# icameling/lidar_camera_calibration

Hardware: AMD Instinct MI355X
Metric: chessboard-corner frames/sec + max corner error (mm), VLP-16 cloud (higher is better)
Workload: dtype f32

## Files before the change

### include/ilcc_hip.h

```cpp
#ifndef ILCC_HIP_H_
#define ILCC_HIP_H_

#include <stdint.h>

#ifdef __cplusplus
extern "C" {
#endif

#define ILCC_MAX_CORNERS 256
#define ILCC_ABI_VERSION 5

enum {
  ILCC_OK = 0,
  ILCC_NO_ROI_POINTS = 1,
  ILCC_NO_CLUSTER = 2,
  ILCC_NO_PLANE = 3,
  ILCC_DEGENERATE_HIST = 4,
  ILCC_TOO_FEW_POINTS = 5,
  ILCC_BAD_ARGUMENT = 6,
  ILCC_CAPACITY = 7,
  ILCC_HIP_ERROR = 8,
  ILCC_IO_ERROR = 9,
  ILCC_BOARD_NOT_FOUND = 10,
  ILCC_AMBIGUOUS = 11
// ... 151 lines not shown
int64_t ilcc_fetch_walk(ilcc_handle* h, uint32_t frame, float* out_yz, uint8_t* out_label, uint64_t cap_points,
                        uint32_t counts[2]);

int32_t ilcc_grid_cost(ilcc_handle* h, const float* yz, const uint8_t* label, uint32_t m,
                       int32_t use_oob, float* cost_out, int32_t* best_index, float* best_cost);

int32_t ilcc_grid_solve(ilcc_handle* h, const float* yz, const uint8_t* label, uint32_t m, int32_t* grid_index, float* grid_cost,
                        int32_t lat[3], int32_t* phase, int64_t* cost_q, int64_t* alt_cost_q, int32_t* rounds, int32_t* hops,
                        int32_t* flags, int32_t* ties);

int32_t ilcc_pattern_refine(ilcc_handle* h, const float* yz, const uint8_t* label, uint32_t m, int32_t lat[3],
                            int32_t* phase, int64_t* cost_q, int64_t* alt_cost_q, int32_t* rounds, int32_t* hops);

int32_t ilcc_get_theta_t(ilcc_handle* h, const float* yz, const uint8_t* label, uint32_t m,
                         int32_t topleft_white, int32_t use_oob, double theta_t[3], double* cost,
                         int32_t* iterations);

#define ILCC_SOLVE_REC_DOUBLES 6
#define ILCC_SOLVE_REC_INTS 4
int32_t ilcc_debug_reference_solve(ilcc_handle* h, const float* yz, const uint8_t* label, const uint64_t* offsets,
                                   const int32_t* status_in, uint32_t n_frames, double* rec_f64, int32_t* rec_i32,
                                   ilcc_result* results, uint32_t* lds_points);

#define ILCC_TIMELINE_COLS 15
int32_t ilcc_debug_timeline_enable(ilcc_handle* h, int32_t on);
int32_t ilcc_debug_timeline_fetch(ilcc_handle* h, double* rows, uint32_t cap_rows);

int32_t ilcc_debug_separate_launches(ilcc_handle* h, int32_t on);

#define ILCC_CLUSTER_HOME_RULE 0
#define ILCC_CLUSTER_HOME_LDS 1
#define ILCC_CLUSTER_HOME_L2 2
#define ILCC_CLUSTER_LAUNCH_WORDS 6
int32_t ilcc_debug_cluster_home(ilcc_handle* h, int32_t home);
int32_t ilcc_debug_cluster_launch(const ilcc_handle* h, uint32_t out[ILCC_CLUSTER_LAUNCH_WORDS]);

int32_t ilcc_debug_group_prepass(ilcc_handle* h, uint32_t* states_out, uint32_t* mask_out, uint32_t dims_out[2], uint32_t* bound_out);
int64_t ilcc_debug_solve_walk(ilcc_handle* h, float* out_yz, uint8_t* out_label, uint64_t cap_points, uint32_t counts[2]);

void ilcc_get_timing(const ilcc_handle* h, ilcc_timing* t);
void ilcc_reset_timing(ilcc_handle* h);

int32_t ilcc_save_corners2txt(const float* corners_xyz, uint32_t n_corners, const char* filename);
int32_t ilcc_read_lidar_corners(const char* filename, uint32_t num, double* out_xyz);

#ifdef __cplusplus
// ... 4 lines not shown
```

### lidar_camera_calibration_amd/_native.py

```python
from __future__ import annotations

import ctypes as C
import os

import numpy as np

_HERE = os.path.dirname(os.path.abspath(__file__))
LIB_PATH = os.environ.get("ILCC_HIP_LIB") or os.path.join(_HERE, "libilcc_hip.so")
MAX_CORNERS = 256

OK, NO_ROI_POINTS, NO_CLUSTER, NO_PLANE, DEGENERATE_HIST, TOO_FEW_POINTS, BAD_ARGUMENT, CAPACITY, \
    HIP_ERROR, IO_ERROR, BOARD_NOT_FOUND, AMBIGUOUS = range(12)
FLAG_TIE_OVERFLOW, FLAG_REFINE_CAPPED, FLAG_LOW_COVERAGE, FLAG_BORDER_RISK = 1, 2, 4, 8
FLAGS_FP32_ONLY = FLAG_TIE_OVERFLOW | FLAG_BORDER_RISK
RECORD_HEADER = 20
TIMELINE_COLS = 15
COST_Q_ONE = float(1 << 40)
SOLVER_REFERENCE_LOCAL, SOLVER_GRID = 0, 1
CLOUD_ROI, CLOUD_CLUSTER, CLOUD_CHESSBOARD, CLOUD_PCA, CLOUD_OPTIM = range(5)

EXPORTS = [
    "ilcc_abi_version", "ilcc_strerror", "ilcc_last_error", "ilcc_default_params",
    "ilcc_set_chessboard_param", "ilcc_create", "ilcc_destroy", "ilcc_set_params", "ilcc_reserve", "ilcc_extract",
    "ilcc_extract_batch", "ilcc_extract_batch_device", "ilcc_submit_batch_device", "ilcc_submit_batch", "ilcc_wait", "ilcc_wait_records_device", "ilcc_fetch_cloud", "ilcc_fetch_labelled", "ilcc_fetch_walk", "ilcc_chessboard_by_point_batch", "ilcc_submit_chessboard_by_point", "ilcc_wait_chessboard_by_point", "ilcc_fetch_classes",
    "ilcc_grid_cost", "ilcc_grid_solve", "ilcc_pattern_refine", "ilcc_get_theta_t", "ilcc_get_timing", "ilcc_reset_timing",
    "ilcc_save_corners2txt", "ilcc_read_lidar_corners",
    "ilcc_set_result_mode", "ilcc_wait_compact", "ilcc_record_floats", "ilcc_fetch_results",
    "ilcc_debug_timeline_enable", "ilcc_debug_timeline_fetch", "ilcc_debug_separate_launches",
    "ilcc_debug_cluster_home", "ilcc_debug_cluster_launch", "ilcc_debug_reference_solve",
    "ilcc_debug_group_prepass", "ilcc_debug_solve_walk",
]
ABI_VERSION = 5
RESULTS_FULL, RESULTS_COMPACT = 0, 1
CLUSTER_HOME_RULE, CLUSTER_HOME_LDS, CLUSTER_HOME_L2 = 0, 1, 2
CLUSTER_LAUNCH_WORDS = 6
SOLVE_REC_DOUBLES, SOLVE_REC_INTS = 6, 4


class Params(C.Structure):
    _fields_ = [
        ("roi_half", C.c_double * 3),
        ("cluster_tol", C.c_double),
        ("cluster_min", C.c_int32),
        ("cluster_max", C.c_int32),
        ("ransac_thresh", C.c_double),
        ("ransac_hyp", C.c_int32),
        ("ransac_seed", C.c_uint32),
        ("hist_bins", C.c_int32),
        ("gray_rate", C.c_double),
        ("huber_delta", C.c_double),
        ("grid_length", C.c_double),
        ("board_w", C.c_int32),
        ("board_h", C.c_int32),
# ... 152 lines not shown
        L.ilcc_wait_compact.restype = C.c_int32
        L.ilcc_record_floats.argtypes = [vp, C.c_int32]
        L.ilcc_record_floats.restype = C.c_uint32
        L.ilcc_debug_timeline_enable.argtypes = [vp, C.c_int32]
        L.ilcc_debug_timeline_enable.restype = C.c_int32
        L.ilcc_debug_timeline_fetch.argtypes = [vp, C.POINTER(C.c_double), C.c_uint32]
        L.ilcc_debug_timeline_fetch.restype = C.c_int32
        if hasattr(L, "ilcc_debug_separate_launches"):
            L.ilcc_debug_separate_launches.argtypes = [vp, C.c_int32]
            L.ilcc_debug_separate_launches.restype = C.c_int32
        if hasattr(L, "ilcc_debug_cluster_home"):
            L.ilcc_debug_cluster_home.argtypes = [vp, C.c_int32]
            L.ilcc_debug_cluster_home.restype = C.c_int32
            L.ilcc_debug_cluster_launch.argtypes = [vp, C.POINTER(C.c_uint32)]
            L.ilcc_debug_cluster_launch.restype = C.c_int32
        L.ilcc_debug_reference_solve.argtypes = [vp, fp, C.POINTER(C.c_uint8), C.POINTER(C.c_uint64), C.POINTER(C.c_int32), C.c_uint32,
                                                 C.POINTER(C.c_double), C.POINTER(C.c_int32), rp, C.POINTER(C.c_uint32)]
        L.ilcc_debug_reference_solve.restype = C.c_int32
        if hasattr(L, "ilcc_debug_group_prepass"):
            L.ilcc_debug_group_prepass.argtypes = [vp, C.POINTER(C.c_uint32), C.POINTER(C.c_uint32), C.POINTER(C.c_uint32), C.POINTER(C.c_uint32)]
            L.ilcc_debug_group_prepass.restype = C.c_int32
            L.ilcc_debug_solve_walk.argtypes = [vp, fp, C.POINTER(C.c_uint8), C.c_uint64, C.POINTER(C.c_uint32)]
            L.ilcc_debug_solve_walk.restype = C.c_int64
        L.ilcc_fetch_results.argtypes = [vp, C.c_uint32, C.c_uint32, rp]
        L.ilcc_fetch_results.restype = C.c_int32
        _lib = L
    return _lib


def default_params() -> Params:
    p = Params()
    lib().ilcc_default_params(C.byref(p))
    return p


def strerror(status: int) -> str:
    return lib().ilcc_strerror(int(status)).decode()


def fptr(a: np.ndarray):
    return a.ctypes.data_as(C.POINTER(C.c_float))
```

### lidar_camera_calibration_amd/csrc/ilcc_api.cpp

```cpp
#include <hip/hip_runtime.h>

#include <array>
#include <cmath>
#include <cstdio>
#include <cstdlib>
#include <cstring>
#include <mutex>
#include <new>
#include <string>
#include <vector>

#include "ilcc_internal.h"
#include "k15_seed.h"
#include "k6_common.h"
#include "k7_common.h"

using namespace ilcc;

namespace ilcc {
bool params_ok(const ilcc_params& p, std::string& why);
}

#ifndef ILCC_SLOTS
#define ILCC_SLOTS 4
// ... 551 lines not shown

GridPass anchor_pass(const ilcc_handle* h, const Ctx& c, const GridSeed& seed, GridPartial* out) {
  GridPass g = whole_grid_pass(c, h->grid, out);
  g.seed = seed;
  g.radius_th = kAnchorRadius;
  g.blocks = 2 * kAnchorRadius + 1;
  return g;
}

GridPass full_pass(const ilcc_handle* h, const Ctx& c, const GridSeed& seed) {
  GridPass g = whole_grid_pass(c, h->grid, c.partial);
  g.seed = seed;
  g.collect_ties = 1u;
  return g;
}

LocatePlan locate_plan(const ilcc_handle* h, const Slot& sl, const Ctx& c) {
  LocatePlan lp{};
  lp.seed = h->seed_grid;
  lp.map = h->seed_map;
  lp.refine_radius = std::max(1, h->seed_map.stride_th / ILCC_REFINE_RADIUS_DIV);
  lp.sample_min = (uint32_t)ILCC_SEED_POINTS;
  lp.sample_cap = std::max((uint32_t)ILCC_SEED_POINTS, ((c.grid_lds_points >> 3) + 63u) & ~63u);
  lp.out = sl.d_partial4;
  return lp;
}

int32_t enqueue_locate_launches(ilcc_handle* h, Slot& sl, const Ctx& c, hipStream_t s, int32_t refine_radius, GridSeed& located) {
  launch_grid_cost(c, seed_pass(h, sl, c), s, 1, nullptr, true);
  HIP_TRY(h, hipEventRecord(sl.ev[kEvSeeded], s));
  const GridPass refine = refine_pass(h, sl, c, refine_radius);
  launch_grid_cost(c, refine, s, 1, nullptr, true);
  HIP_TRY(h, hipEventRecord(sl.ev[kEvRefined], s));
  located = full_table_records(refine.out, refine.blocks);
  GridPartial* const ping[2] = {sl.d_partial4, sl.d_partial2};
  for (int round = 0; round < kAnchorRounds; ++round) {
    const GridPass anchor = anchor_pass(h, c, located, ping[round & 1]);
    launch_anchor(c, anchor, s);
    located = full_table_records(anchor.out, anchor.blocks);
  }
  return ILCC_OK;
}

int32_t enqueue_grid_search(ilcc_handle* h, Slot& sl, const Ctx& c, hipStream_t s, uint32_t n_frames, bool chain, bool walk_laid_out = false) {
  const bool prune = h->p.grid_prune != 0;
  if (!walk_laid_out) launch_walk_order(c, s);
  HIP_TRY(h, hipEventRecord(sl.ev[kEvWalkOrdered], s));
  GridSeed located{};
  if (h->seed_grid.n_th > 0 && h->p.n_th >= 8 && h->p.n_ty >= 8 && h->p.n_tz >= 8) {
    const LocatePlan lp = locate_plan(h, sl, c);
    const bool fused = n_frames >= (uint32_t)kLocateMinFrames && lp.seed.n_th <= 16 &&
                       locate_lds_bytes(lp.sample_cap, h->grid.n_ty, h->grid.n_tz, lp.seed.n_ty, lp.seed.n_tz) <= (size_t)kLocateLdsMax;
    if (fused) {
      launch_locate(c, s, lp);
      HIP_TRY(h, hipEventRecord(sl.ev[kEvSeeded], s));
      HIP_TRY(h, hipEventRecord(sl.ev[kEvRefined], s));
      located = full_table_records(lp.out, 1);
    } else {
      ILCC_TRY(enqueue_locate_launches(h, sl, c, s, lp.refine_radius, located));
    }
  } else {
    HIP_TRY(h, hipEventRecord(sl.ev[kEvSeeded], s));
    HIP_TRY(h, hipEventRecord(sl.ev[kEvRefined], s));
  }
  HIP_TRY(h, hipEventRecord(sl.ev[kEvAnchored], s));
  GridPass full = full_pass(h, c, located);
  const GroupPrepassPlan gp = group_prepass_plan(h->p);
  full.box_points = gp.box ? (uint32_t)ILCC_BOX_POINTS : 0u;
  if (full.box_points != 0u && gp.on && (size_t)n_frames * gp.groups <= sl.grp_alive_cap &&
      (size_t)n_frames * gp.groups * gp.words <= sl.grp_mask_cap) {
    full.grp_alive = sl.d_grp_alive;
    full.grp_mask = sl.d_grp_mask;
    full.grp_count = gp.groups;
    full.grp_words = gp.words;
    launch_group_prepass(c, full, s);
// ... 835 lines not shown
    HIP_TRY(h, hipMemcpyAsync(sl.d_lab, label, total, hipMemcpyHostToDevice, s));
  }
  HIP_TRY(h, hipMemsetAsync(sl.d_solverec, 0xFF, sizeof(SolveRec) * 2 * n_frames, s));
  sl.n_frames = 0;
  const Ctx c = make_ctx(h, sl, nullptr, nullptr, n_frames, 1);
  launch_reference_solve(c, s);
  launch_corners(c, s, solve_slots(c.p));
  HIP_TRY(h, hipGetLastError());
  std::vector<SolveRec> rec(2 * (size_t)n_frames);
  HIP_TRY(h, hipMemcpyAsync(rec.data(), sl.d_solverec, sizeof(SolveRec) * rec.size(), hipMemcpyDeviceToHost, s));
  HIP_TRY(h, hipMemcpyAsync(results, sl.d_res, sizeof(ilcc_result) * n_frames, hipMemcpyDeviceToHost, s));
  ILCC_TRY(sync_own(h, s));
  for (size_t k = 0; k < rec.size(); ++k) {
    const SolveRec& r = rec[k];
    const double d[ILCC_SOLVE_REC_DOUBLES] = {r.x[0], r.x[1], r.x[2], r.cost_a, r.cost_b, r.sel};
    const int32_t i[ILCC_SOLVE_REC_INTS] = {r.iters_a, r.iters_b, r.phase, r.valid};
    std::memcpy(rec_f64 + ILCC_SOLVE_REC_DOUBLES * k, d, sizeof(d));
    std::memcpy(rec_i32 + ILCC_SOLVE_REC_INTS * k, i, sizeof(i));
  }
  if (lds_points) *lds_points = c.grid_lds_points;
  return ILCC_OK;
}

int32_t ilcc_pattern_refine(ilcc_handle* h, const float* yz, const uint8_t* label, uint32_t m, int32_t lat[3],
                            int32_t* phase, int64_t* cost_q, int64_t* alt_cost_q, int32_t* rounds, int32_t* hops) {
  if (!h || !lat || !phase) return ILCC_BAD_ARGUMENT;
  if (lat[0] < h->th_lat_lo || lat[0] > h->th_lat_hi || (*phase != 0 && *phase != 1)) {
    h->err = "ilcc_pattern_refine: theta lattice coordinate outside [th_min - refine_th_margin, th_max + refine_th_margin] steps";
    return ILCC_BAD_ARGUMENT;
  }
  const hipStream_t s = h->stream[take_stream(h)];
  ILCC_TRY(stage_labelled(h, s, yz, label, m));
  Slot& sl = h->slots[0];
  RefineOut io{};
  io.lat[0] = lat[0];
  io.lat[1] = lat[1];
  io.lat[2] = lat[2];
  io.phase = *phase;
  HIP_TRY(h, hipMemcpyAsync(h->d_refine_io, &io, sizeof(io), hipMemcpyHostToDevice, s));
  const Ctx c = diagnostic_ctx(h, sl, 0);
  launch_pattern_refine_test(c, s, h->d_refine_io);
  HIP_TRY(h, hipGetLastError());
  HIP_TRY(h, hipMemcpyAsync(&io, h->d_refine_io, sizeof(io), hipMemcpyDeviceToHost, s));
  ILCC_TRY(sync_own(h, s));
  lat[0] = io.lat[0];
  lat[1] = io.lat[1];
// ... 98 lines not shown
```

### lidar_camera_calibration_amd/csrc/ilcc_internal.h

```cpp
#pragma once

#include <hip/hip_runtime.h>
#include <stdint.h>

#include "ilcc_hip.h"

#define ILCC_WAVE 64

namespace ilcc {

constexpr int kCuLdsBytes = 160 * 1024;
constexpr int kClusterLdsMax = kCuLdsBytes - 4 * 1024;
constexpr int kLocateLdsMax = 3 * (kCuLdsBytes / 8);
constexpr int kSolveLdsMax = kCuLdsBytes - 16 * 1024;

constexpr int kCropThreads = 256;
constexpr int kCropChunk = 4096;
#ifndef ILCC_K2_THREADS
#define ILCC_K2_THREADS 256
#endif
constexpr int kFrameThreads = ILCC_K2_THREADS;
#ifndef ILCC_K3_THREADS
#define ILCC_K3_THREADS 256
#endif
// ... 221 lines not shown
__device__ __forceinline__ uint32_t block_rank(bool flag, uint32_t* scratch, uint32_t& total) {
  const unsigned long long m = __ballot(flag);
  const int lane = lane_id();
  const uint32_t in_wave = __popcll(m & ((1ull << lane) - 1ull));
  const int nw = (blockDim.x + ILCC_WAVE - 1) / ILCC_WAVE;
  __syncthreads();
  if (lane == 0) scratch[wave_id()] = __popcll(m);
  __syncthreads();
  uint32_t base = 0, tot = 0;
  for (int w = 0; w < nw; ++w) {
    const uint32_t c = scratch[w];
    if (w < wave_id()) base += c;
    tot += c;
  }
  total = tot;
  return base + in_wave;
}

struct LocatePlan {
  GridTables seed;
  SeedMap map;
  int32_t refine_radius;
  uint32_t sample_min, sample_cap;
  GridPartial* out;
};

size_t locate_lds_bytes(uint32_t sample_cap, int n_ty, int n_tz, int n_ty2, int n_tz2);
void launch_locate(const Ctx& c, hipStream_t s, const LocatePlan& lp);
void launch_anchor(const Ctx& c, const GridPass& pass, hipStream_t s);
constexpr int kRefineThetaStride = 2;
constexpr int kLocateMinFrames = 512;

void launch_roi_crop(const Ctx& c, hipStream_t s, hipEvent_t after_count = nullptr, bool one_pass = false);
constexpr int kCropFrameMinFrames = 512;
constexpr int32_t kClusterHomeRule = 0, kClusterHomeLds = 1, kClusterHomeL2 = 2;
struct ClusterLimits {
  uint32_t cus, lds_per_cu, threads_per_cu, static_lds;
};
struct ClusterLaunch {
  int32_t home;
  uint32_t lds_bytes, threads;
};
hipError_t cluster_limits(int device, ClusterLimits* out);
ClusterLaunch launch_cluster(const Ctx& c, hipStream_t s, const ClusterLimits& lim, int32_t home);
void launch_cluster_listed(const Ctx& c, hipStream_t s);
constexpr size_t kListedFrameBytes = 64;
hipError_t set_kernel_attributes_k2();
size_t cluster_lds_bytes(uint32_t pts_cap, uint32_t cells_cap, uint32_t bits);
uint32_t cluster_bits_default();
uint32_t cluster_bits_online();
// ... 25 lines not shown
```

### lidar_camera_calibration_amd/csrc/k6_locate.hip

```cpp
#include "k6_common.h"

namespace ilcc {

__device__ __forceinline__ void anchor_walk(const ilcc_params& p, const GridTables& t, const FrameWalk& fw, int k, int a_org, int b_org, const float* ty, const float* tz,
                                            uint32_t part, uint32_t n_parts, float (*s_part)[2], uint32_t& pts_done, uint32_t& pts_in) {
  const int my_s = lane_id() & (kSlices - 1), my_c = lane_id() >> 2;
  const float Wh = 0.5f * (float)p.board_w, Hh = 0.5f * (float)p.board_h, delta2 = (float)p.huber_delta;
  const float cth = t.cth[k], sth = t.sth[k];
  const float ay = ty[min(a_org + (my_c >> 2), t.n_ty - 1)], az = tz[min(b_org + (my_c & 3), t.n_tz - 1)];
  float A0 = 0.f, A1 = 0.f;
  uint32_t pos = 0, pin = 0;
  for (uint32_t at0 = part * kSlices; at0 < fw.M; at0 += n_parts * kSlices) {
    const uint32_t at = at0 + (uint32_t)my_s;
    if (at < fw.M) {
      const uint32_t src = fw.source(at, fw.Mi_all, fw.n_rim_all);
      const float2 v = rotate(fw.yz[src], cth, sth);
      const PointTerms pt{v.x, v.y, fw.lab[src] ? 0.5f : 0.f};
      if (at < fw.Mi_all)
        accumulate_interior(pt, ay, az, delta2, A0, A1);
      else
        accumulate<true>(pt, ay, az, Wh, Hh, delta2, A0, A1);
    }
    pos += kSlices;
    pin += at0 < fw.Mi_all ? (uint32_t)kSlices : 0u;
  }
  pts_done += pos;
  pts_in += pin;
  const float t0s = quad_sum(A0), t1s = quad_sum(A1);
  if (my_s == 0) {
    s_part[my_c][0] = t0s;
    s_part[my_c][1] = t1s;
  }
}

template <int THETAS, int PARTS>
__device__ __forceinline__ void anchor_publish(const GridTables& t, uint32_t* bound, const float (*s_part)[16][2], int k0, int a_org, int b_org,
                                               GridPartial* out) {
  const int lane = lane_id();
  const int n_ty = t.n_ty, n_tz = t.n_tz;
  Best best{__builtin_inff(), 0xFFFFFFFFu, 0xFFFFFFFFu};
  uint32_t ab = 0;
  if (lane < 16 * THETAS) {
    const int th = lane >> 4, cand = lane & 15;
    const int k = min(max(k0 + th, 0), t.n_th - 1), ja = a_org + (cand >> 2), jb = b_org + (cand & 3);
    if (ja < n_ty && jb < n_tz) {
      float h0 = 0.f, h1 = 0.f;
#pragma unroll
      for (int q = 0; q < PARTS; ++q) {
        h0 += s_part[th * PARTS + q][cand][0];
        h1 += s_part[th * PARTS + q][cand][1];
      }
      score(2.f * h0, 2.f * h1, k, ja, jb, n_ty, n_tz, t.c_th, t.c_ty, t.c_tz, best, ab);
    }
  }
  best = wave_argmin<true>(best, ab);
  if (lane == 0) {
    *out = GridPartial{best.cost, best.d2, best.flat, ab};
    if (best.flat != 0xFFFFFFFFu) atomicMin(bound, __float_as_uint(best.cost));
  }
}

constexpr int kLocateThreads = 384;
constexpr int kSeedPeek = 16;
constexpr int kAnchorThetas = 3;
constexpr int kAnchorParts = (kLocateThreads / 64) / kAnchorThetas;
constexpr int kLocateWaves = kLocateThreads / ILCC_WAVE;
constexpr int kLocateThetasMax = 16;
constexpr int kLocateWindowTiles = 2;

struct LocateLds {
  size_t hw, rot, ay, az, ay2, az2, bytes;
};
__host__ __device__ constexpr LocateLds locate_lds(uint32_t sample_cap, int n_ty, int n_tz, int n_ty2, int n_tz2) {
  LocateLds l{};
  l.hw = sizeof(float2) * (size_t)sample_cap;
  l.rot = l.hw + sizeof(float) * (size_t)sample_cap;
  l.ay = l.rot + sizeof(float2) * (size_t)kLocateThetasMax * sample_cap;
  l.az = l.ay + sizeof(float) * (size_t)n_ty;
  l.ay2 = l.az + sizeof(float) * (size_t)n_tz;
  l.az2 = l.ay2 + sizeof(float) * (size_t)n_ty2;
  l.bytes = l.az2 + sizeof(float) * (size_t)n_tz2;
  return l;
}
size_t locate_lds_bytes(uint32_t sample_cap, int n_ty, int n_tz, int n_ty2, int n_tz2) { return locate_lds(sample_cap, n_ty, n_tz, n_ty2, n_tz2).bytes; }

__global__ __launch_bounds__(kLocateThreads) void k6_locate(Ctx c, LocatePlan lp) {
  extern __shared__ __align__(16) unsigned char smem[];
  __shared__ Best s_best[kLocateWaves];
  __shared__ uint32_t s_ab[kLocateWaves];
  __shared__ uint32_t s_bound;
  __shared__ uint32_t s_pick[4];
  __shared__ uint32_t s_iters[kLocateWaves], s_iters_in[kLocateWaves];
  __shared__ float s_part[kAnchorThetas * kAnchorParts][16][2];
  const uint32_t f = blockIdx.x;
  GridPartial* out = lp.out + f;
  const int lane = lane_id();
  const int wid = __builtin_amdgcn_readfirstlane(wave_id());
  if (c.res[f].status != ILCC_OK) {
    if (threadIdx.x == 0) no_candidate(out);
    return;
  }
  const FrameWalk fw(c, f);
  const uint32_t Ms = min(fw.sample(lp.sample_min), lp.sample_cap);
  uint32_t n_in, n_rm;
  fw.prefix(Ms, n_in, n_rm);
  const GridTables& full = c.grid;
  const int n_ty = full.n_ty, n_tz = full.n_tz, n_th = full.n_th;
  const int n_ty2 = lp.seed.n_ty, n_tz2 = lp.seed.n_tz;
  const LocateLds l = locate_lds(lp.sample_cap, n_ty, n_tz, n_ty2, n_tz2);
  float2* s_raw = reinterpret_cast<float2*>(smem);
  float* s_hw = lds_next<float>(s_raw, 0, l.hw);
  float2* s_rot = lds_next<float2>(s_hw, l.hw, l.rot);
  float* s_ay = lds_next<float>(s_rot, l.rot, l.ay);
  float* s_az = lds_next<float>(s_ay, l.ay, l.az);
  float* s_ay2 = lds_next<float>(s_az, l.az, l.ay2);
  float* s_az2 = lds_next<float>(s_ay2, l.ay2, l.az2);
  for (uint32_t sl = threadIdx.x; sl < Ms; sl += kLocateThreads) {
    const uint32_t src = fw.source(sl, n_in, n_rm);
    s_raw[sl] = fw.yz[src];
    s_hw[sl] = fw.lab[src] ? 0.5f : 0.f;
  }
  for (int i = threadIdx.x; i < n_ty; i += kLocateThreads) s_ay[i] = full.ay[i];
  for (int i = threadIdx.x; i < n_tz; i += kLocateThreads) s_az[i] = full.az[i];
  for (int i = threadIdx.x; i < n_ty2; i += kLocateThreads) s_ay2[i] = lp.seed.ay[i];
  for (int i = threadIdx.x; i < n_tz2; i += kLocateThreads) s_az2[i] = lp.seed.az[i];
  if (threadIdx.x == 0) s_bound = 0x7f800000u;
  const float Wh = 0.5f * (float)c.p.board_w, Hh = 0.5f * (float)c.p.board_h, delta2 = (float)c.p.huber_delta;
  const int my_s = lane & (kSlices - 1), my_c = lane >> 2, my_a = my_c >> 2, my_b = my_c & 3;
  uint32_t pts_done = 0, pts_in = 0;

  auto rotate_sample = [&](int n_rot, auto th_of, const float* cth_tab, const float* sth_tab) {
    for (uint32_t item = threadIdx.x; item < (uint32_t)n_rot * Ms; item += kLocateThreads) {
      const uint32_t r = item / Ms, sl = item - r * Ms;
      const int k = th_of((int)r);
      s_rot[(size_t)r * lp.sample_cap + sl] = rotate(s_raw[sl], cth_tab[k], sth_tab[k]);
// ... 49 lines not shown
  };
  auto reduce_best = [&](Best best, uint32_t ab) {
    best = wave_argmin<true>(best, ab);
    if (lane == 0) {
      s_best[wid] = best;
      s_ab[wid] = ab;
    }
    __syncthreads();
    if (threadIdx.x == 0) {
      uint32_t bab = 0;
      const Best b = block_argmin<kLocateWaves>(s_best, s_ab, bab);
      s_pick[0] = b.flat;
      s_pick[1] = bab;
      s_pick[2] = __float_as_uint(b.cost);
      s_pick[3] = b.d2;
    }
    __syncthreads();
  };
  auto lower_sample_bound = [&](float v) {
    const float wb = wave_min(v);
    if (lane == 0) atomicMin(&s_bound, __float_as_uint(wb));
  };
  __syncthreads();

  const int n_th2 = min(lp.seed.n_th, kLocateThetasMax);
  rotate_sample(n_th2, [&](int r) { return r; }, lp.seed.cth, lp.seed.sth);
  __syncthreads();
  {
    const int nta = axis_tiles(n_ty2), ntb = axis_tiles(n_tz2), per = nta * ntb, n_tiles = n_th2 * per;
    Best best{__builtin_inff(), 0xFFFFFFFFu, 0xFFFFFFFFu};
    uint32_t best_ab = 0;
    int t_first = -1;
    {
      float peek_best = __builtin_inff();
      for (int t = wid; t < n_tiles; t += kLocateWaves) {
        const int k2 = t / per, q = t - k2 * per, ta = q / ntb, tb = q - ta * ntb;
        const int ia = ta * kTile + my_a, ib = tb * kTile + my_b;
        const float2* rot = s_rot + (size_t)k2 * lp.sample_cap;
        const float ay = s_ay2[min(ia, n_ty2 - 1)], az = s_az2[min(ib, n_tz2 - 1)];
        float A0 = 0.f, A1 = 0.f;
        for (uint32_t at0 = n_in; at0 < min(Ms, n_in + (uint32_t)kSeedPeek); at0 += kSlices) {
          const uint32_t at = at0 + (uint32_t)my_s;
          if (at < Ms) {
            const float2 v = rot[at];
            accumulate<true>(PointTerms{v.x, v.y, s_hw[at]}, ay, az, Wh, Hh, delta2, A0, A1);
          }
        }
        pts_done += min(Ms - n_in, (uint32_t)kSeedPeek);
        const float pm = wave_min((ia < n_ty2 && ib < n_tz2) ? fminf(quad_sum(A0), quad_sum(A1)) : __builtin_inff());
        if (pm < peek_best) {
          peek_best = pm;
          t_first = t;
        }
      }
    }
    const int n_mine = (n_tiles - wid + kLocateWaves - 1) / kLocateWaves;
    for (int it = (t_first >= 0 ? -1 : 0); it < n_mine; ++it) {
      const int t = it < 0 ? t_first : wid + it * kLocateWaves;
      if (it >= 0 && t == t_first) continue;
      const int k2 = t / per, q = t - k2 * per, ta = q / ntb, tb = q - ta * ntb;
      const int ia = ta * kTile + my_a, ib = tb * kTile + my_b;
      const bool owner = ia < n_ty2 && ib < n_tz2;
      float c0, c1;
      if (!sample_tile(s_rot + (size_t)k2 * lp.sample_cap, s_ay2[min(ia, n_ty2 - 1)], s_az2[min(ib, n_tz2 - 1)], c0, c1)) continue;
      if (owner) score(c0, c1, k2, ia, ib, n_ty2, n_tz2, lp.seed.c_th, lp.seed.c_ty, lp.seed.c_tz, best, best_ab);
      lower_sample_bound(owner ? fminf(c0, c1) : __builtin_inff());
    }
    reduce_best(best, best_ab);
  }
  if (s_pick[0] == 0xFFFFFFFFu) {
    if (threadIdx.x == 0) no_candidate(out);
    return;
  }
  const int k2s = (int)((s_pick[0] >> 1) / (uint32_t)(n_ty2 * n_tz2));
  const int sa = min((int)(s_pick[1] >> 16) * lp.map.stride_t, n_ty - 1), sbb = min((int)(s_pick[1] & 0xFFFFu) * lp.map.stride_t, n_tz - 1);
  constexpr int kRefStride = kRefineThetaStride;
  const int n_ref = min(2 * (lp.refine_radius / kRefStride) + 1, kLocateThetasMax);
  const int k_ref0 = lp.map.off_th + k2s * lp.map.stride_th - (lp.refine_radius / kRefStride) * kRefStride;
  rotate_sample(n_ref, [&](int r) { return min(max(k_ref0 + kRefStride * r, 0), n_th - 1); }, full.cth, full.sth);
  __syncthreads();
  {
    constexpr int kWindow = kLocateWindowTiles * kTile;
    const int a_org = window_origin(sa, kWindow / 2, n_ty, kWindow), b_org = window_origin(sbb, kWindow / 2, n_tz, kWindow);
    const int nta = min(kLocateWindowTiles, axis_tiles(n_ty)), ntb = min(kLocateWindowTiles, axis_tiles(n_tz));
    const int per = nta * ntb, n_tiles = n_ref * per;
    Best best{__builtin_inff(), 0xFFFFFFFFu, 0xFFFFFFFFu};
    uint32_t best_ab = 0;
    for (int t = wid; t < n_tiles; t += kLocateWaves) {
      const int r = t / per, q = t - r * per, ta = q / ntb, tb = q - ta * ntb;
      const int k = min(max(k_ref0 + kRefStride * r, 0), n_th - 1);
      const int ia = a_org + ta * kTile + my_a, ib = b_org + tb * kTile + my_b;
      const bool owner = ia < n_ty && ib < n_tz;
      float c0, c1;
      if (!sample_tile(s_rot + (size_t)r * lp.sample_cap, s_ay[min(ia, n_ty - 1)], s_az[min(ib, n_tz - 1)], c0, c1)) continue;
      if (owner) score(c0, c1, k, ia, ib, n_ty, n_tz, full.c_th, full.c_ty, full.c_tz, best, best_ab);
      lower_sample_bound(owner ? fminf(c0, c1) : __builtin_inff());
    }
    reduce_best(best, best_ab);
  }
  {
    const int kr = (int)((s_pick[0] >> 1) / (uint32_t)(n_ty * n_tz));
    const int ra = min((int)(s_pick[1] >> 16), n_ty - 1), rb = min((int)(s_pick[1] & 0xFFFFu), n_tz - 1);
    const int a_org = window_origin(ra, 1, n_ty, kTile), b_org = window_origin(rb, 1, n_tz, kTile);
    const int k0 = kr - kAnchorThetas / 2;
    if (wid < kAnchorThetas * kAnchorParts) {
      const int t = wid % kAnchorThetas, part = wid / kAnchorThetas;
      anchor_walk(c.p, full, fw, min(max(k0 + t, 0), n_th - 1), a_org, b_org, s_ay, s_az, (uint32_t)part, kAnchorParts, s_part[t * kAnchorParts + part],
                  pts_done, pts_in);
    }
    __syncthreads();
    if (wid == 0) anchor_publish<kAnchorThetas, kAnchorParts>(full, c.grid_bound + f, s_part, k0, a_org, b_org, out);
  }
  if (lane == 0) {
    s_iters[wid] = pts_done;
    s_iters_in[wid] = pts_in;
  }
  __syncthreads();
  if (threadIdx.x == 0) {
    uint32_t it_sum = 0, in_sum = 0;
    for (int w = 0; w < kLocateWaves; ++w) {
      it_sum += s_iters[w];
      in_sum += s_iters_in[w];
    }
    count_evals(c.grid_iters, f, kEvalsAll, it_sum);
    count_evals(c.grid_iters, f, kEvalsInterior, in_sum);
  }
}

constexpr int kAnchorThreads = 512;
constexpr int kAnchorWaves = kAnchorThreads / ILCC_WAVE;
__global__ __launch_bounds__(kAnchorThreads) void k6_anchor(Ctx c, GridPass pass) {
  __shared__ float s_part[kAnchorWaves][16][2];
  __shared__ uint32_t s_iters[kAnchorWaves], s_iters_in[kAnchorWaves];
  const uint32_t f = blockIdx.y, kblk = blockIdx.x;
  GridPartial* out = &pass.out[(uint64_t)f * pass.blocks + kblk];
  const int lane = lane_id();
  const int wid = __builtin_amdgcn_readfirstlane(wave_id());
  uint32_t k2u = 0, ab = 0;
  Best sb{__builtin_inff(), 0xFFFFFFFFu, 0xFFFFFFFFu};
  if (c.res[f].status == ILCC_OK) sb = seed_argmin(pass.seed, f, k2u, ab);
  if (sb.flat == 0xFFFFFFFFu) {
    if (threadIdx.x == 0) no_candidate(out);
    return;
  }
  const int n_ty = pass.t.n_ty, n_tz = pass.t.n_tz;
  const int kr = (int)((sb.flat >> 1) / (uint32_t)(n_ty * n_tz));
  const int k0 = kr + (int)kblk - pass.radius_th;
  const int ra = min((int)(ab >> 16), n_ty - 1), rb = min((int)(ab & 0xFFFFu), n_tz - 1);
  const int a_org = window_origin(ra, 1, n_ty, kTile), b_org = window_origin(rb, 1, n_tz, kTile);
  uint32_t pts_done = 0, pts_in = 0;
  anchor_walk(c.p, pass.t, FrameWalk(c, f), min(max(k0, 0), pass.t.n_th - 1), a_org, b_org, pass.t.ay, pass.t.az, (uint32_t)wid, kAnchorWaves, s_part[wid], pts_done,
              pts_in);
  if (lane == 0) {
    s_iters[wid] = pts_done;
    s_iters_in[wid] = pts_in;
  }
  __syncthreads();
  if (wid == 0) anchor_publish<1, kAnchorWaves>(pass.t, pass.bound + f, s_part, k0, a_org, b_org, out);
  if (threadIdx.x == 0) {
    uint32_t it_sum = 0, in_sum = 0;
    for (int w = 0; w < kAnchorWaves; ++w) {
      it_sum += s_iters[w];
      in_sum += s_iters_in[w];
    }
    count_evals(c.grid_iters, f, kEvalsAll, it_sum);
    count_evals(c.grid_iters, f, kEvalsInterior, in_sum);
  }
}

void launch_anchor(const Ctx& c, const GridPass& pass, hipStream_t s) {
  hipLaunchKernelGGL(k6_anchor, dim3(pass.blocks, c.n_frames), dim3(kAnchorThreads), 0, s, c, pass);
}

void launch_locate(const Ctx& c, hipStream_t s, const LocatePlan& lp) {
  const size_t lds = locate_lds_bytes(lp.sample_cap, c.grid.n_ty, c.grid.n_tz, lp.seed.n_ty, lp.seed.n_tz);
  hipLaunchKernelGGL(k6_locate, dim3(c.n_frames), dim3(kLocateThreads), lds, s, c, lp);
}

hipError_t set_kernel_attributes_k6_locate() { return raise_grid_lds_limit({(const void*)k6_locate}); }

}
```

Measured before the change: 1.336 million.

## Stage frame points in LDS for fused locate anchor walk with batched loads

In the fused locate kernel, the anchor walk's frame points and half-white labels are now copied once into LDS, reusing the rotation buffer, when the frame fits. All anchor waves then read from LDS instead of re-reading global memory. The anchor walk is templated over its point source and split into interior, mixed and border trip ranges, with loads batched four ahead to raise memory-level parallelism and drop per-point branches. The change also adds a debug locate entry point and optional cycle-counter profiling, and it may enlarge the LDS request, which can cut occupancy or push some grids off the fused path.

```diff
diff --git a/include/ilcc_hip.h b/include/ilcc_hip.h
--- a/include/ilcc_hip.h
+++ b/include/ilcc_hip.h
@@ -197,6 +197,9 @@
                                    const int32_t* status_in, uint32_t n_frames, double* rec_f64, int32_t* rec_i32,
                                    ilcc_result* results, uint32_t* lds_points);
 
+int32_t ilcc_debug_locate(ilcc_handle* h, const float* yz, const uint8_t* label, const uint64_t* offsets, uint32_t n_frames,
+                          uint32_t* records_out, uint32_t* bound_out);
+
 #define ILCC_TIMELINE_COLS 15
 int32_t ilcc_debug_timeline_enable(ilcc_handle* h, int32_t on);
 int32_t ilcc_debug_timeline_fetch(ilcc_handle* h, double* rows, uint32_t cap_rows);
diff --git a/lidar_camera_calibration_amd/_native.py b/lidar_camera_calibration_amd/_native.py
--- a/lidar_camera_calibration_amd/_native.py
+++ b/lidar_camera_calibration_amd/_native.py
@@ -28,7 +28,7 @@
     "ilcc_set_result_mode", "ilcc_wait_compact", "ilcc_record_floats", "ilcc_fetch_results",
     "ilcc_debug_timeline_enable", "ilcc_debug_timeline_fetch", "ilcc_debug_separate_launches",
     "ilcc_debug_cluster_home", "ilcc_debug_cluster_launch", "ilcc_debug_reference_solve",
-    "ilcc_debug_group_prepass", "ilcc_debug_solve_walk",
+    "ilcc_debug_group_prepass", "ilcc_debug_solve_walk", "ilcc_debug_locate",
 ]
 ABI_VERSION = 5
 RESULTS_FULL, RESULTS_COMPACT = 0, 1
@@ -227,6 +227,10 @@
             L.ilcc_debug_group_prepass.restype = C.c_int32
             L.ilcc_debug_solve_walk.argtypes = [vp, fp, C.POINTER(C.c_uint8), C.c_uint64, C.POINTER(C.c_uint32)]
             L.ilcc_debug_solve_walk.restype = C.c_int64
+        if hasattr(L, "ilcc_debug_locate"):
+            L.ilcc_debug_locate.argtypes = [vp, fp, C.POINTER(C.c_uint8), C.POINTER(C.c_uint64), C.c_uint32, C.POINTER(C.c_uint32),
+                                            C.POINTER(C.c_uint32)]
+            L.ilcc_debug_locate.restype = C.c_int32
         L.ilcc_fetch_results.argtypes = [vp, C.c_uint32, C.c_uint32, rp]
         L.ilcc_fetch_results.restype = C.c_int32
         _lib = L
diff --git a/lidar_camera_calibration_amd/csrc/ilcc_api.cpp b/lidar_camera_calibration_amd/csrc/ilcc_api.cpp
--- a/lidar_camera_calibration_amd/csrc/ilcc_api.cpp
+++ b/lidar_camera_calibration_amd/csrc/ilcc_api.cpp
@@ -597,6 +597,7 @@
   lp.refine_radius = std::max(1, h->seed_map.stride_th / ILCC_REFINE_RADIUS_DIV);
   lp.sample_min = (uint32_t)ILCC_SEED_POINTS;
   lp.sample_cap = std::max((uint32_t)ILCC_SEED_POINTS, ((c.grid_lds_points >> 3) + 63u) & ~63u);
+  lp.stage_cap = ILCC_LOCATE_STAGE_ANCHOR ? c.grid_lds_points : 0u;
   lp.out = sl.d_partial4;
   return lp;
 }
@@ -625,7 +626,7 @@
   if (h->seed_grid.n_th > 0 && h->p.n_th >= 8 && h->p.n_ty >= 8 && h->p.n_tz >= 8) {
     const LocatePlan lp = locate_plan(h, sl, c);
     const bool fused = n_frames >= (uint32_t)kLocateMinFrames && lp.seed.n_th <= 16 &&
-                       locate_lds_bytes(lp.sample_cap, h->grid.n_ty, h->grid.n_tz, lp.seed.n_ty, lp.seed.n_tz) <= (size_t)kLocateLdsMax;
+                       locate_lds_bytes(lp, h->grid.n_ty, h->grid.n_tz) <= (size_t)kLocateLdsMax;
     if (fused) {
       launch_locate(c, s, lp);
       HIP_TRY(h, hipEventRecord(sl.ev[kEvSeeded], s));
@@ -1507,6 +1508,60 @@
   return ILCC_OK;
 }
 
+int32_t ilcc_debug_locate(ilcc_handle* h, const float* yz, const uint8_t* label, const uint64_t* offsets, uint32_t n_frames,
+                          uint32_t* records_out, uint32_t* bound_out) {
+  if (!h || !records_out || !bound_out) return ILCC_BAD_ARGUMENT;
+  Slot& sl = h->slots[0];
+  if (sl.busy) {
+    h->err = "diagnostic entry while ticket 0 is in flight";
+    return ILCC_BAD_ARGUMENT;
+  }
+  if (h->p.solver != ILCC_SOLVER_GRID) {
+    h->err = "ilcc_debug_locate needs ILCC_SOLVER_GRID";
+    return ILCC_BAD_ARGUMENT;
+  }
+  ILCC_TRY(check_offsets(h, offsets, n_frames));
+  const uint64_t total = offsets[n_frames];
+  if (total > 0 && (!yz || !label)) return ILCC_BAD_ARGUMENT;
+  HIP_TRY(h, hipSetDevice(h->device));
+  const Ctx c = make_ctx(h, sl, nullptr, nullptr, n_frames, 1);
+  const LocatePlan lp = locate_plan(h, sl, c);
+  if (!(h->seed_grid.n_th > 0 && h->p.n_th >= 8 && h->p.n_ty >= 8 && h->p.n_tz >= 8) || lp.seed.n_th > 16 ||
+      locate_lds_bytes(lp, h->grid.n_ty, h->grid.n_tz) > (size_t)kLocateLdsMax) {
+    h->err = "ilcc_debug_locate: this grid (or LDS capacity) does not take k6_locate";
+    return ILCC_CAPACITY;
+  }
+  const hipStream_t s = h->stream[take_stream(h)];
+  std::vector<uint32_t> n_lab(n_frames), stride(n_frames), bound(n_frames, 0x7f800000u);
+  std::vector<ilcc_result> res(n_frames);
+  std::memset(res.data(), 0, sizeof(ilcc_result) * n_frames);
+  for (uint32_t f = 0; f < n_frames; ++f) {
+    n_lab[f] = (uint32_t)(offsets[f + 1] - offsets[f]);
+    stride[f] = walk_stride(n_lab[f]);
+    res[f].status = ILCC_OK;
+  }
+  HIP_TRY(h, hipMemcpyAsync(sl.d_off, offsets, sizeof(uint64_t) * (n_frames + 1), hipMemcpyHostToDevice, s));
+  HIP_TRY(h, hipMemcpyAsync(sl.d_res, res.data(), sizeof(ilcc_result) * n_frames, hipMemcpyHostToDevice, s));
+  HIP_TRY(h, hipMemcpyAsync(sl.d_nlab, n_lab.data(), sizeof(uint32_t) * n_frames, hipMemcpyHostToDevice, s));
+  HIP_TRY(h, hipMemcpyAsync(sl.d_walk, stride.data(), sizeof(uint32_t) * n_frames, hipMemcpyHostToDevice, s));
+  HIP_TRY(h, hipMemcpyAsync(sl.d_bound, bound.data(), sizeof(uint32_t) * n_frames, hipMemcpyHostToDevice, s));
+  HIP_TRY(h, hipMemsetAsync(sl.d_iters, 0, sizeof(unsigned long long) * kBatchWords, s));
+  if (total > 0) {
+    HIP_TRY(h, hipMemcpyAsync(sl.d_yz, yz, sizeof(float2) * total, hipMemcpyHostToDevice, s));
+    HIP_TRY(h, hipMemcpyAsync(sl.d_lab, label, total, hipMemcpyHostToDevice, s));
+  }
+  HIP_TRY(h, hipMemsetAsync(lp.out, 0xFF, sizeof(GridPartial) * n_frames, s));
+  sl.n_frames = 0;
+  launch_walk_order(c, s);
+  launch_locate(c, s, lp);
+  HIP_TRY(h, hipGetLastError());
+  static_assert(sizeof(GridPartial) == 4 * sizeof(uint32_t), "records_out: four words per frame");
+  HIP_TRY(h, hipMemcpyAsync(records_out, lp.out, sizeof(GridPartial) * n_frames, hipMemcpyDeviceToHost, s));
+  HIP_TRY(h, hipMemcpyAsync(bound_out, sl.d_bound, sizeof(uint32_t) * n_frames, hipMemcpyDeviceToHost, s));
+  ILCC_TRY(sync_own(h, s));
+  return ILCC_OK;
+}
+
 int32_t ilcc_pattern_refine(ilcc_handle* h, const float* yz, const uint8_t* label, uint32_t m, int32_t lat[3],
                             int32_t* phase, int64_t* cost_q, int64_t* alt_cost_q, int32_t* rounds, int32_t* hops) {
   if (!h || !lat || !phase) return ILCC_BAD_ARGUMENT;
diff --git a/lidar_camera_calibration_amd/csrc/ilcc_internal.h b/lidar_camera_calibration_amd/csrc/ilcc_internal.h
--- a/lidar_camera_calibration_amd/csrc/ilcc_internal.h
+++ b/lidar_camera_calibration_amd/csrc/ilcc_internal.h
@@ -267,10 +267,14 @@
   SeedMap map;
   int32_t refine_radius;
   uint32_t sample_min, sample_cap;
+  uint32_t stage_cap;
   GridPartial* out;
 };
 
-size_t locate_lds_bytes(uint32_t sample_cap, int n_ty, int n_tz, int n_ty2, int n_tz2);
+#ifndef ILCC_LOCATE_STAGE_ANCHOR
+#define ILCC_LOCATE_STAGE_ANCHOR 1
+#endif
+size_t locate_lds_bytes(const LocatePlan& lp, int n_ty, int n_tz);
 void launch_locate(const Ctx& c, hipStream_t s, const LocatePlan& lp);
 void launch_anchor(const Ctx& c, const GridPass& pass, hipStream_t s);
 constexpr int kRefineThetaStride = 2;
diff --git a/lidar_camera_calibration_amd/csrc/k6_locate.hip b/lidar_camera_calibration_amd/csrc/k6_locate.hip
--- a/lidar_camera_calibration_amd/csrc/k6_locate.hip
+++ b/lidar_camera_calibration_amd/csrc/k6_locate.hip
@@ -1,36 +1,121 @@
 #include "k6_common.h"
 
+#ifdef ILCC_K6_TIMING
+#include <algorithm>
+#include <vector>
+#endif
+
 namespace ilcc {
 
-__device__ __forceinline__ void anchor_walk(const ilcc_params& p, const GridTables& t, const FrameWalk& fw, int k, int a_org, int b_org, const float* ty, const float* tz,
-                                            uint32_t part, uint32_t n_parts, float (*s_part)[2], uint32_t& pts_done, uint32_t& pts_in) {
+#ifdef ILCC_K6_TIMING
+constexpr int kLocateProfWaves = 1 << 14, kLocateProfWords = 8;
+__device__ unsigned long long k6_locate_prof[kLocateProfWaves * kLocateProfWords];
+#define K6L_STAMP(name) const unsigned long long name = __builtin_readcyclecounter()
+#else
+#define K6L_STAMP(name)
+#endif
+
+struct WalkStaged {
+  using Label = float;
+  const float2* yz;
+  const float* half_white;
+  __device__ __forceinline__ void load(uint32_t at, float2& v, Label& l) const {
+    v = yz[at];
+    l = half_white[at];
+  }
+  __device__ __forceinline__ float hw(Label l) const { return l; }
+};
+template <bool LAYOUT>
+struct WalkGlobal {
+  using Label = uint8_t;
+  const float2* __restrict__ yz;
+  const uint8_t* __restrict__ lab;
+  uint32_t M, S;
+  __device__ __forceinline__ explicit WalkGlobal(const FrameWalk& fw) : yz(fw.yz), lab(fw.lab), M(fw.M), S(fw.S) {}
+  __device__ __forceinline__ void load(uint32_t at, float2& v, Label& l) const {
+    const uint32_t src = LAYOUT ? at : (uint32_t)(((uint64_t)at * S) % M);
+    v = yz[src];
+    l = lab[src];
+  }
+  __device__ __forceinline__ float hw(Label l) const { return l ? 0.5f : 0.f; }
+};
+
+constexpr int kAnchorAhead = 4;
+template <class Source>
+__device__ __forceinline__ void anchor_walk(const ilcc_params& p, const GridTables& t, const Source& src, uint32_t M, uint32_t Mi_all, int k, int a_org, int b_org,
+                                            const float* ty, const float* tz, uint32_t part, uint32_t n_parts, float (*s_part)[2], uint32_t& pts_done,
+                                            uint32_t& pts_in) {
   const int my_s = lane_id() & (kSlices - 1), my_c = lane_id() >> 2;
   const float Wh = 0.5f * (float)p.board_w, Hh = 0.5f * (float)p.board_h, delta2 = (float)p.huber_delta;
   const float cth = t.cth[k], sth = t.sth[k];
   const float ay = ty[min(a_org + (my_c >> 2), t.n_ty - 1)], az = tz[min(b_org + (my_c & 3), t.n_tz - 1)];
   float A0 = 0.f, A1 = 0.f;
-  uint32_t pos = 0, pin = 0;
-  for (uint32_t at0 = part * kSlices; at0 < fw.M; at0 += n_parts * kSlices) {
-    const uint32_t at = at0 + (uint32_t)my_s;
-    if (at < fw.M) {
-      const uint32_t src = fw.source(at, fw.Mi_all, fw.n_rim_all);
-      const float2 v = rotate(fw.yz[src], cth, sth);
-      const PointTerms pt{v.x, v.y, fw.lab[src] ? 0.5f : 0.f};
-      if (at < fw.Mi_all)
-        accumulate_interior(pt, ay, az, delta2, A0, A1);
-      else
-        accumulate<true>(pt, ay, az, Wh, Hh, delta2, A0, A1);
-    }
-    pos += kSlices;
-    pin += at0 < fw.Mi_all ? (uint32_t)kSlices : 0u;
-  }
-  pts_done += pos;
-  pts_in += pin;
+  const uint32_t first = part * kSlices, stride = n_parts * kSlices;
+  auto trips_below = [&](uint32_t x) { return x > first ? (x - first + stride - 1u) / stride : 0u; };
+  const uint32_t n_in = trips_below(Mi_all & ~(uint32_t)(kSlices - 1));
+  const uint32_t n_mix = trips_below(Mi_all);
+  const uint32_t n_bd = max(n_mix, trips_below(M & ~(uint32_t)(kSlices - 1)));
+  const uint32_t n_all = trips_below(M);
+  auto term = [&](auto interior, const float2 raw, float hw) {
+    const float2 v = rotate(raw, cth, sth);
+    const PointTerms pt{v.x, v.y, hw};
+    if constexpr (decltype(interior)::value)
+      accumulate_interior(pt, ay, az, delta2, A0, A1);
+    else
+      accumulate<true>(pt, ay, az, Wh, Hh, delta2, A0, A1);
+  };
+  auto whole_trips = [&](uint32_t t0, uint32_t t1, auto interior) {
+    uint32_t tr = t0;
+    for (; tr + (uint32_t)kAnchorAhead <= t1; tr += kAnchorAhead) {
+      float2 v[kAnchorAhead];
+      typename Source::Label l[kAnchorAhead];
+#pragma unroll
+      for (int e = 0; e < kAnchorAhead; ++e) src.load(first + (tr + (uint32_t)e) * stride + (uint32_t)my_s, v[e], l[e]);
+#pragma unroll
+      for (int e = 0; e < kAnchorAhead; ++e) term(interior, v[e], src.hw(l[e]));
+    }
+    if (tr < t1) {
+      float2 v[kAnchorAhead - 1];
+      typename Source::Label l[kAnchorAhead - 1];
+#pragma unroll
+      for (int e = 0; e < kAnchorAhead - 1; ++e) src.load(first + min(tr + (uint32_t)e, t1 - 1u) * stride + (uint32_t)my_s, v[e], l[e]);
+#pragma unroll
+      for (int e = 0; e < kAnchorAhead - 1; ++e)
+        if (tr + (uint32_t)e < t1) term(interior, v[e], src.hw(l[e]));
+    }
+  };
+  auto tested_trips = [&](uint32_t t0, uint32_t t1) {
+    for (uint32_t tr = t0; tr < t1; ++tr) {
+      const uint32_t at = first + tr * stride + (uint32_t)my_s;
+      if (at < M) {
+        float2 v;
+        typename Source::Label l;
+        src.load(at, v, l);
+        if (at < Mi_all)
+          term(std::true_type{}, v, src.hw(l));
+        else
+          term(std::false_type{}, v, src.hw(l));
+      }
+    }
+  };
+  whole_trips(0u, n_in, std::true_type{});
+  tested_trips(n_in, n_mix);
+  whole_trips(n_mix, n_bd, std::false_type{});
+  tested_trips(n_bd, n_all);
+  pts_done += n_all * (uint32_t)kSlices;
+  pts_in += n_mix * (uint32_t)kSlices;
   const float t0s = quad_sum(A0), t1s = quad_sum(A1);
   if (my_s == 0) {
     s_part[my_c][0] = t0s;
     s_part[my_c][1] = t1s;
   }
+}
+template <class... Rest>
+__device__ __forceinline__ void anchor_walk_global(const ilcc_params& p, const GridTables& t, const FrameWalk& fw, Rest&&... rest) {
+  if (fw.layout)
+    anchor_walk(p, t, WalkGlobal<true>(fw), fw.M, fw.Mi_all, rest...);
+  else
+    anchor_walk(p, t, WalkGlobal<false>(fw), fw.M, 0u, rest...);
 }
 
 template <int THETAS, int PARTS>
@@ -66,23 +151,28 @@
 constexpr int kAnchorParts = (kLocateThreads / 64) / kAnchorThetas;
 constexpr int kLocateWaves = kLocateThreads / ILCC_WAVE;
 constexpr int kLocateThetasMax = 16;
+constexpr int kStageAhead = 8;
 constexpr int kLocateWindowTiles = 2;
 
 struct LocateLds {
-  size_t hw, rot, ay, az, ay2, az2, bytes;
+  size_t hw, rot, stage_hw, ay, az, ay2, az2, bytes;
 };
-__host__ __device__ constexpr LocateLds locate_lds(uint32_t sample_cap, int n_ty, int n_tz, int n_ty2, int n_tz2) {
+__host__ __device__ constexpr LocateLds locate_lds(uint32_t sample_cap, uint32_t stage_cap, int n_ty, int n_tz, int n_ty2, int n_tz2) {
   LocateLds l{};
   l.hw = sizeof(float2) * (size_t)sample_cap;
   l.rot = l.hw + sizeof(float) * (size_t)sample_cap;
-  l.ay = l.rot + sizeof(float2) * (size_t)kLocateThetasMax * sample_cap;
+  l.stage_hw = l.rot + sizeof(float2) * (size_t)stage_cap;
+  const size_t rotations = sizeof(float2) * (size_t)kLocateThetasMax * sample_cap, staged = (sizeof(float2) + sizeof(float)) * (size_t)stage_cap;
+  l.ay = l.rot + (rotations > staged ? rotations : staged);
   l.az = l.ay + sizeof(float) * (size_t)n_ty;
   l.ay2 = l.az + sizeof(float) * (size_t)n_tz;
   l.az2 = l.ay2 + sizeof(float) * (size_t)n_ty2;
   l.bytes = l.az2 + sizeof(float) * (size_t)n_tz2;
   return l;
 }
-size_t locate_lds_bytes(uint32_t sample_cap, int n_ty, int n_tz, int n_ty2, int n_tz2) { return locate_lds(sample_cap, n_ty, n_tz, n_ty2, n_tz2).bytes; }
+size_t locate_lds_bytes(const LocatePlan& lp, int n_ty, int n_tz) {
+  return locate_lds(lp.sample_cap, lp.stage_cap, n_ty, n_tz, lp.seed.n_ty, lp.seed.n_tz).bytes;
+}
 
 __global__ __launch_bounds__(kLocateThreads) void k6_locate(Ctx c, LocatePlan lp) {
   extern __shared__ __align__(16) unsigned char smem[];
@@ -94,6 +184,7 @@
   __shared__ float s_part[kAnchorThetas * kAnchorParts][16][2];
   const uint32_t f = blockIdx.x;
   GridPartial* out = lp.out + f;
+  K6L_STAMP(t_entry);
   const int lane = lane_id();
   const int wid = __builtin_amdgcn_readfirstlane(wave_id());
   if (c.res[f].status != ILCC_OK) {
@@ -107,10 +198,11 @@
   const GridTables& full = c.grid;
   const int n_ty = full.n_ty, n_tz = full.n_tz, n_th = full.n_th;
   const int n_ty2 = lp.seed.n_ty, n_tz2 = lp.seed.n_tz;
-  const LocateLds l = locate_lds(lp.sample_cap, n_ty, n_tz, n_ty2, n_tz2);
+  const LocateLds l = locate_lds(lp.sample_cap, lp.stage_cap, n_ty, n_tz, n_ty2, n_tz2);
   float2* s_raw = reinterpret_cast<float2*>(smem);
   float* s_hw = lds_next<float>(s_raw, 0, l.hw);
   float2* s_rot = lds_next<float2>(s_hw, l.hw, l.rot);
+  float* s_stage_hw = lds_next<float>(s_rot, l.rot, l.stage_hw);
   float* s_ay = lds_next<float>(s_rot, l.rot, l.ay);
   float* s_az = lds_next<float>(s_ay, l.ay, l.az);
   float* s_ay2 = lds_next<float>(s_az, l.az, l.ay2);
@@ -206,6 +298,7 @@
     if (lane == 0) atomicMin(&s_bound, __float_as_uint(wb));
   };
   __syncthreads();
+  K6L_STAMP(t_staged);
 
   const int n_th2 = min(lp.seed.n_th, kLocateThetasMax);
   rotate_sample(n_th2, [&](int r) { return r; }, lp.seed.cth, lp.seed.sth);
@@ -252,6 +345,7 @@
     }
     reduce_best(best, best_ab);
   }
+  K6L_STAMP(t_seeded);
   if (s_pick[0] == 0xFFFFFFFFu) {
     if (threadIdx.x == 0) no_candidate(out);
     return;
@@ -282,18 +376,66 @@
     }
     reduce_best(best, best_ab);
   }
+  K6L_STAMP(t_refined);
   {
     const int kr = (int)((s_pick[0] >> 1) / (uint32_t)(n_ty * n_tz));
     const int ra = min((int)(s_pick[1] >> 16), n_ty - 1), rb = min((int)(s_pick[1] & 0xFFFFu), n_tz - 1);
     const int a_org = window_origin(ra, 1, n_ty, kTile), b_org = window_origin(rb, 1, n_tz, kTile);
     const int k0 = kr - kAnchorThetas / 2;
+    const bool staged = fw.layout && fw.M <= lp.stage_cap;
+    if (staged) {
+      auto stage = [&](uint32_t base, auto ahead) {
+        constexpr int N = decltype(ahead)::value;
+        float2 v[N];
+        uint8_t lb[N];
+#pragma unroll
+        for (int e = 0; e < N; ++e) {
+          const uint32_t i = min(base + (uint32_t)e * kLocateThreads + threadIdx.x, fw.M - 1u);
+          v[e] = fw.yz[i];
+          lb[e] = fw.lab[i];
+        }
+#pragma unroll
+        for (int e = 0; e < N; ++e) {
+          const uint32_t i = base + (uint32_t)e * kLocateThreads + threadIdx.x;
+          if (i < fw.M) {
+            s_rot[i] = v[e];
+            s_stage_hw[i] = lb[e] ? 0.5f : 0.f;
+          }
+        }
+      };
+      for (uint32_t base = 0; base < fw.M; base += (uint32_t)kStageAhead * kLocateThreads) {
+        if (fw.M - base <= (uint32_t)(kStageAhead / 2) * kLocateThreads)
+          stage(base, std::integral_constant<int, kStageAhead / 2>{});
+        else
+          stage(base, std::integral_constant<int, kStageAhead>{});
+      }
+      __syncthreads();
+    }
+    K6L_STAMP(t_copied);
     if (wid < kAnchorThetas * kAnchorParts) {
-      const int t = wid % kAnchorThetas, part = wid / kAnchorThetas;
-      anchor_walk(c.p, full, fw, min(max(k0 + t, 0), n_th - 1), a_org, b_org, s_ay, s_az, (uint32_t)part, kAnchorParts, s_part[t * kAnchorParts + part],
-                  pts_done, pts_in);
+      const int t = wid % kAnchorThetas, part = wid / kAnchorThetas, k = min(max(k0 + t, 0), n_th - 1);
+      float(*my_part)[2] = s_part[t * kAnchorParts + part];
+      if (staged)
+        anchor_walk(c.p, full, WalkStaged{s_rot, s_stage_hw}, fw.M, fw.Mi_all, k, a_org, b_org, s_ay, s_az, (uint32_t)part, (uint32_t)kAnchorParts, my_part, pts_done,
+                    pts_in);
+      else
+        anchor_walk_global(c.p, full, fw, k, a_org, b_org, s_ay, s_az, (uint32_t)part, (uint32_t)kAnchorParts, my_part, pts_done, pts_in);
     }
     __syncthreads();
     if (wid == 0) anchor_publish<kAnchorThetas, kAnchorParts>(full, c.grid_bound + f, s_part, k0, a_org, b_org, out);
+#ifdef ILCC_K6_TIMING
+    if (lane == 0) {
+      const unsigned long long t_anchored = __builtin_readcyclecounter();
+      unsigned long long* o = k6_locate_prof + (size_t)((f * kLocateWaves + (uint32_t)wid) & (kLocateProfWaves - 1)) * kLocateProfWords;
+      o[0] = 1ull;
+      o[1] = t_staged - t_entry;
+      o[2] = t_seeded - t_staged;
+      o[3] = t_refined - t_seeded;
+      o[4] = t_copied - t_refined;
+      o[5] = t_anchored - t_copied;
+      o[6] = t_anchored - t_entry;
+    }
+#endif
   }
   if (lane == 0) {
     s_iters[wid] = pts_done;
@@ -333,8 +475,8 @@
   const int ra = min((int)(ab >> 16), n_ty - 1), rb = min((int)(ab & 0xFFFFu), n_tz - 1);
   const int a_org = window_origin(ra, 1, n_ty, kTile), b_org = window_origin(rb, 1, n_tz, kTile);
   uint32_t pts_done = 0, pts_in = 0;
-  anchor_walk(c.p, pass.t, FrameWalk(c, f), min(max(k0, 0), pass.t.n_th - 1), a_org, b_org, pass.t.ay, pass.t.az, (uint32_t)wid, kAnchorWaves, s_part[wid], pts_done,
-              pts_in);
+  anchor_walk_global(c.p, pass.t, FrameWalk(c, f), min(max(k0, 0), pass.t.n_th - 1), a_org, b_org, pass.t.ay, pass.t.az, (uint32_t)wid, (uint32_t)kAnchorWaves, s_part[wid],
+                     pts_done, pts_in);
   if (lane == 0) {
     s_iters[wid] = pts_done;
     s_iters_in[wid] = pts_in;
@@ -357,10 +499,25 @@
 }
 
 void launch_locate(const Ctx& c, hipStream_t s, const LocatePlan& lp) {
-  const size_t lds = locate_lds_bytes(lp.sample_cap, c.grid.n_ty, c.grid.n_tz, lp.seed.n_ty, lp.seed.n_tz);
+  const size_t lds = locate_lds_bytes(lp, c.grid.n_ty, c.grid.n_tz);
   hipLaunchKernelGGL(k6_locate, dim3(c.n_frames), dim3(kLocateThreads), lds, s, c, lp);
 }
 
+#ifdef ILCC_K6_TIMING
+extern "C" int ilcc_debug_k6_locate_profile(unsigned long long* out8, int clear) {
+  static std::vector<unsigned long long> host((size_t)kLocateProfWaves * kLocateProfWords);
+  if (hipMemcpyFromSymbol(host.data(), HIP_SYMBOL(k6_locate_prof), host.size() * sizeof(unsigned long long)) != hipSuccess) return -1;
+  for (int k = 0; k < kLocateProfWords; ++k) out8[k] = 0;
+  for (size_t w = 0; w < (size_t)kLocateProfWaves; ++w)
+    for (int k = 0; k < kLocateProfWords; ++k) out8[k] += host[w * kLocateProfWords + k];
+  if (clear) {
+    std::fill(host.begin(), host.end(), 0ull);
+    if (hipMemcpyToSymbol(HIP_SYMBOL(k6_locate_prof), host.data(), host.size() * sizeof(unsigned long long)) != hipSuccess) return -1;
+  }
+  return 0;
+}
+#endif
+
 hipError_t set_kernel_attributes_k6_locate() { return raise_grid_lds_limit({(const void*)k6_locate}); }
 
 }
```

Result: faster. 1.401 million (median of 6 runs) (+4.9%).
